# google-research/corenet

Hardware: AMD Instinct MI355X
Metric: voxels/sec fwd+bwd @128^3 (higher is better)
Workload: dtype bf16x3 (the convolutions of decoder stages 3-6 and the encoder's 3x3 convolutions -- forward of stages 4-5, data gradient of all -- multiply operands split into two bf16 terms: three bf16 MFMAs per product, fp32 accumulation, 16 mantissa bits, ~3e-6 relative per layer; tensors, everything else and t

## Files before the change

### corenet_amd/_lib.py

```python
from __future__ import annotations

import ctypes as C
import os
from typing import Optional

import torch as t

_HERE = os.path.dirname(os.path.abspath(__file__))
TOOLS_LIB_PATH = os.path.join(os.path.dirname(_HERE), "tools", "_build", "libcorenet_hip_tools.so")
PROBE_LIB_PATH = os.path.join(os.path.dirname(_HERE), "tools", "_build", "libcrn_probe.so")
LIB_PATH = os.environ.get("CORENET_HIP_LIB", TOOLS_LIB_PATH if os.environ.get("CRN_TOOLS_LIB") == "1" else
                          os.path.join(_HERE, "lib", "libcorenet_hip.so"))

c_i32p = C.POINTER(C.c_int32)
c_f32p = C.c_void_p
vp = C.c_void_p
i64 = C.c_int64
i32 = C.c_int
f32 = C.c_float
sz = C.c_size_t


class CrnTapBoxes(C.Structure):
  _fields_ = [("n_groups", C.c_int32), ("c_groups", C.c_int32), ("n_box", (C.c_int8 * 6) * 8),
# ... 32 lines not shown
  _fields_ = [("scale", vp), ("shift", vp), ("pre_relu", C.c_int32), ("post_relu", C.c_int32)]


class CrnBnBwdFuse(C.Structure):
  _fields_ = [("x", vp), ("sB_x", i64), ("saved", vp), ("pre_relu", C.c_int32), ("ws", vp), ("ws_bytes", sz),
              ("dsum", vp), ("ndsum", C.c_int32), ("nparts", C.c_int32)]


class HipError(RuntimeError):
  pass


_SIGS = {
    "crn_conv_fwd": [C.POINTER(CrnView), C.POINTER(CrnInTransform), vp, i32, vp, i32,
                     C.POINTER(CrnView), i32, i32, i32, i32, i32, i32, i32, i32, vp, vp],
    "crn_conv_fwd_plan": [C.POINTER(CrnView), C.POINTER(CrnInTransform), vp, i32, vp, i32,
                          C.POINTER(CrnView), i32, i32, i32, i32, i32, i32, i32, i32, vp, C.POINTER(CrnConvPlan)],
    "crn_conv_wgrad_plan": [C.POINTER(CrnView), C.POINTER(CrnInTransform), C.POINTER(CrnView), vp, i32,
                            i32, i32, i32, i32, i32, i32, i32, vp, C.POINTER(CrnConvPlan)],
    "crn_conv_fwd_bf3": [C.POINTER(CrnView), C.POINTER(CrnInTransform), vp, i32, vp, i32,
                         C.POINTER(CrnView), i32, i32, i32, i32, i32, i32, i32, vp, vp],
    "crn_conv_fwd_bf3_slabs": [C.POINTER(CrnView), C.POINTER(CrnInTransform), vp, i32, vp, i32,
                               C.POINTER(CrnView), i32, i32, i32, i32, i32, i32, i32, vp, vp],
    "crn_conv_fwd_bf3_slabs_bnbwd": [C.POINTER(CrnView), C.POINTER(CrnInTransform), vp, i32, vp, i32,
                                     C.POINTER(CrnView), i32, i32, i32, i32, i32, i32, i32, vp, C.POINTER(CrnBnBwdFuse), vp],
    "crn_conv_fwd_bf3_slabs_stats": [C.POINTER(CrnView), C.POINTER(CrnInTransform), vp, i32, vp, i32,
                                     C.POINTER(CrnView), i32, i32, i32, i32, i32, i32, i32, vp, i32, vp, sz, C.POINTER(C.c_int), vp],
    "crn_batch_renorm_bwd_apply": [vp, i64, vp, i64, i32, i32, i64, i32, vp, vp, vp, vp, vp, i64, vp, vp, i32, vp, i32,
                                   vp, sz, i32, vp],
    "crn_conv_wgrad_bf3": [C.POINTER(CrnView), C.POINTER(CrnInTransform), C.POINTER(CrnView), vp, i32,
# ... 250 lines not shown
```

### corenet_amd/backend.py

```python
from __future__ import annotations

import ctypes as C
from typing import Optional

import torch as t

from corenet_amd import _lib
from corenet_amd._lib import CrnInTransform, CrnView, ptr
from corenet_amd.views import View, space_to_depth_view, view_of

_DTYPE_CODE = {t.float32: 0, t.uint8: 1, t.int32: 2, t.float64: 3, t.int64: 4, t.int16: 5, t.int8: 6}


def _cview(v: View) -> CrnView:
  base = v.storage.data_ptr() + 4 * (v.offset - v.storage.storage_offset())
  c = v.__dict__.get("_crn")
  if c is None or c[0] != base:
    c = (base, CrnView(base, v.B, v.C, v.D, v.H, v.W, v.sB, v.sC, ptr(v.chan_off), v.sD, v.sH, v.sW))
    object.__setattr__(v, "_crn", c)
  return c[1]


class Transform:
  __slots__ = ("scale", "shift", "pre_relu", "post_relu")
# ... 52 lines not shown
               splits: int = 1, accumulate: bool = False, boxes=None, math: str = "fp32", wslab=None):
    if math == "bf16x3" and wslab is not None:
      self.lib.crn_conv_fwd_bf3_slabs(C.byref(_cview(x)), _ctr(tr), ptr(wslab), npad, ptr(bias), bias_sB,
                                      C.byref(_cview(y)), window[0], window[1], window[2],
                                      pad_lo[0], pad_lo[1], pad_lo[2], int(accumulate), _ctapboxes(boxes), _lib.stream())
      return
    if math == "bf16x3":
      self.lib.crn_conv_fwd_bf3(C.byref(_cview(x)), _ctr(tr), ptr(w), npad, ptr(bias), bias_sB,
                                C.byref(_cview(y)), window[0], window[1], window[2],
                                pad_lo[0], pad_lo[1], pad_lo[2], int(accumulate), _ctapboxes(boxes), _lib.stream())
      return
    self.lib.crn_conv_fwd(C.byref(_cview(x)), _ctr(tr), ptr(w), npad, ptr(bias), bias_sB,
                          C.byref(_cview(y)), window[0], window[1], window[2],
                          pad_lo[0], pad_lo[1], pad_lo[2], splits, int(accumulate), _ctapboxes(boxes),
                          _lib.stream())

  @staticmethod
  def _plan_dict(p) -> dict:
    d = {n: int(getattr(p, n)) for n, _ in p._fields_}
    d["path"] = _lib.PLAN_PATHS[d["path"]]
    return d

  def conv_fwd_plan(self, x: View, tr: Optional[Transform], w: t.Tensor, npad: int, bias: Optional[t.Tensor], bias_sB: int,
                    y: View, window, pad_lo, splits: int = 1, accumulate: bool = False, boxes=None) -> dict:
    p = _lib.CrnConvPlan()
    self.lib.crn_conv_fwd_plan(C.byref(_cview(x)), _ctr(tr), ptr(w), npad, ptr(bias), bias_sB, C.byref(_cview(y)),
                               window[0], window[1], window[2], pad_lo[0], pad_lo[1], pad_lo[2], splits, int(accumulate),
                               _ctapboxes(boxes), C.byref(p))
    return self._plan_dict(p)

# ... 452 lines not shown
```

### corenet_amd/csrc/batch_renorm.hip

```cpp
#include "crn_common.h"
#include <cstdlib>
#include <algorithm>
#include <type_traits>

namespace {

constexpr int kThreads = 256;

struct Slice { int64_t s0, s1; };
__device__ __forceinline__ Slice block_slice(int64_t S) {
  int64_t chunk = (S + gridDim.x - 1) / gridDim.x;
  chunk = (chunk + 3) & ~(int64_t)3;
  Slice r;
  r.s0 = (int64_t)blockIdx.x * chunk;
  r.s1 = min(S, r.s0 + chunk);
  return r;
}

template <bool VEC, typename F4, typename F1>
__device__ __forceinline__ void for_slice(Slice sl, F4 f4, F1 f1) {
  if (VEC) {
#pragma unroll 4
    for (int64_t s = sl.s0 + (int64_t)threadIdx.x * 4; s + 3 < sl.s1; s += (int64_t)kThreads * 4) f4(s);
    const int64_t nfull = (sl.s1 > sl.s0) ? ((sl.s1 - sl.s0) & ~(int64_t)3) : 0;
    for (int64_t s = sl.s0 + nfull + threadIdx.x; s < sl.s1; s += kThreads) f1(s);
  } else {
    for (int64_t s = sl.s0 + threadIdx.x; s < sl.s1; s += kThreads) f1(s);
  }
}

__device__ __forceinline__ void bn_acc(float v, int pre_relu, double& s1, double& s2) {
  if (pre_relu) v = fmaxf(v, 0.f);
  s1 += (double)v;
  s2 += (double)v * (double)v;
}

template <bool VEC>
__global__ __launch_bounds__(kThreads) void bn_partial_kernel(const float* x, int64_t S, int64_t sB,
                                                               int pre_relu, double* ws) {
  __shared__ double red[kThreads / 64];
  const int c = blockIdx.y, b = blockIdx.z;
  const float* p = x + (int64_t)b * sB + (int64_t)c * S;
  double s1 = 0.0, s2 = 0.0;
  auto one = [&](float v) { bn_acc(v, pre_relu, s1, s2); };
  for_slice<VEC>(block_slice(S),
                 [&](int64_t s) { const f32x4 v = *reinterpret_cast<const f32x4*>(p + s);
                                  one(v.x); one(v.y); one(v.z); one(v.w); },
                 [&](int64_t s) { one(p[s]); });
  const double t1 = crn_block_sum(s1, red);
  const double t2 = crn_block_sum(s2, red);
  if (threadIdx.x == 0) {
    const int nparts = gridDim.x * gridDim.z;
    double* o = ws + ((int64_t)c * nparts + (int64_t)b * gridDim.x + blockIdx.x) * 2;
    o[0] = t1; o[1] = t2;
  }
}

struct BnChannelIn { float g, bt, rmean, rvar, nt; };
__device__ __forceinline__ BnChannelIn bn_channel_in(int c, const float* gamma, const float* beta,
                                                     const float* running_mean, const float* running_var,
                                                     const int64_t* nbt) {
  return BnChannelIn{gamma[c], beta[c], running_mean[c], running_var[c], (float)nbt[0]};
}
// ... 90 lines not shown
    for_slice<VEC>(all,
                   [&](int64_t s) { const f32x4 v = *reinterpret_cast<const f32x4*>(p + s);
                                    one(v.x); one(v.y); one(v.z); one(v.w); },
                   [&](int64_t s) { one(p[s]); });
  }
  const double t1 = crn_block_sum(s1, red);
  const double t2 = crn_block_sum(s2, red);
  if (threadIdx.x == 0)
    bn_finalize_channel(c, C, t1, t2, (double)B * (double)S, cin, running_mean, running_var, eps, momentum, scale, shift,
                        saved);
}

typedef float f32x2 __attribute__((ext_vector_type(2)));

__device__ __forceinline__ f32x4 bn_splitk_sum(const float* part, int splits, int B, int C, int S4, int b, int c, int s4) {
  const f32x4* pp = reinterpret_cast<const f32x4*>(part) + ((int64_t)b * C + c) * S4 + s4;
  const int64_t slab4 = (int64_t)B * C * S4;
  f32x4 sum = (f32x4){0.f, 0.f, 0.f, 0.f};
  for (int sp = 0; sp < splits; ++sp) sum += pp[sp * slab4];
  return sum;
}

__device__ __forceinline__ bool bn_stride2_offset(int c, int s4, int W, int W2, int H2, int64_t& off) {
  const int s = s4 * 4, row = s / W, col = s - row * W;
  off = ((int64_t)c * H2 + (row >> 1)) * W2 + (col >> 1);
  return !(row & 1);
}

struct BnTail {
  const float* r; const float* rscale; const float* rshift; int64_t sBr;
  float* y_pre; int64_t sBpre; float* y; int64_t sBy; int relu;
  float* y2; int64_t sBy2; int W, W2, H2;
};
template <int NV, bool TAIL = false>
__global__ __launch_bounds__(kThreads) void bn_owner_stats_reg_kernel(
// ... 181 lines not shown
      f32x4 o;
#pragma unroll
      for (int i = 0; i < 4; ++i) {
        o[i] = bn_bwd_dx(xv[k][i], gv[k][i], pre_relu, post_relu, ch, kf, mg, mgx);
        lsum += o[i];
      }
      *reinterpret_cast<f32x4*>(dx + (int64_t)b * sBdx + ((int64_t)c * S4 + s4) * 4) = o;
    }
  }
  if (dsum && c < ndsum) {
    const float tsum = bn_block_sum_f32(lsum, redf);
    if (threadIdx.x == 0) dsum[c] = tsum;
  }
}

template <bool VEC>
__global__ __launch_bounds__(kThreads) void bn_bwd_partial_kernel(
    const float* x, int64_t sBx, const float* dy, int64_t sBdy, int64_t S, int C, int pre_relu,
    int post_relu, const float* scale, const float* shift, const float* saved, double* ws, float* dsum,
    int ndsum) {
  __shared__ double red[kThreads / 64];
  const int c = blockIdx.y, b = blockIdx.z;
  if (dsum && c < ndsum && blockIdx.x == 0 && b == 0 && threadIdx.x == 0) dsum[c] = 0.f;
  const float* px = x + (int64_t)b * sBx + (int64_t)c * S;
  const float* pg = dy + (int64_t)b * sBdy + (int64_t)c * S;
  const BnBwdChannel ch = bn_bwd_channel(c, C, scale, shift, saved);
  double s1 = 0.0, s2 = 0.0;
  auto one = [&](float xv, float gv) { bn_bwd_acc(xv, gv, pre_relu, post_relu, ch, s1, s2); };
  for_slice<VEC>(block_slice(S),
                 [&](int64_t s) { const f32x4 a = *reinterpret_cast<const f32x4*>(px + s);
                                  const f32x4 g = *reinterpret_cast<const f32x4*>(pg + s);
                                  one(a.x, g.x); one(a.y, g.y); one(a.z, g.z); one(a.w, g.w); },
                 [&](int64_t s) { one(px[s], pg[s]); });
  const double t1 = crn_block_sum(s1, red);
  const double t2 = crn_block_sum(s2, red);
  if (threadIdx.x == 0) {
    const int nparts = gridDim.x * gridDim.z;
    double* o = ws + ((int64_t)c * nparts + (int64_t)b * gridDim.x + blockIdx.x) * 2;
    o[0] = t1; o[1] = t2;
  }
}

template <bool VEC>
__global__ __launch_bounds__(kThreads) void bn_bwd_apply_kernel(
    const float* x, int64_t sBx, const float* dy, int64_t sBdy, int64_t S, int C, int pre_relu,
    int post_relu, const float* gamma, const float* scale, const float* shift, const float* saved,
    const double* ws, int nparts, double count, float* dx, int64_t sBdx, float* dgamma,
    float* dbeta, int accumulate, float* dsum, int ndsum) {
// ... 208 lines not shown

constexpr int kMaxParts = 64 * 64;

template <typename F>
inline void with_nv(int64_t BS, F f) {
  const int per = (int)crn_cdiv(BS / 4, kThreads);
  if (per <= 1) f(std::integral_constant<int, 1>{}); else if (per <= 2) f(std::integral_constant<int, 2>{});
  else if (per <= 4) f(std::integral_constant<int, 4>{}); else if (per <= 8) f(std::integral_constant<int, 8>{});
  else f(std::integral_constant<int, 16>{});
}
template <typename F>
inline void with_bool(bool on, F f) {
  if (on) f(std::true_type{}); else f(std::false_type{});
}

int take_or_flush_pending(const float* base, int64_t sB, int B, int C, int64_t S, hipStream_t st, bool reg_form,
                          const float** part, int* splits) {
  *part = nullptr; *splits = 0;
  CrnSplitPending& pend = crn_splitk_pending();
  if (!pend.active) return CRN_OK;
  const crnView& py = pend.y;
  if (reg_form && pend.stream == st && py.base == base && py.B == B && py.C == C && (int64_t)py.D * py.H * py.W == S && sB == (int64_t)C * S) {
    *part = pend.scratch; *splits = pend.splits; pend.active = false;
    return CRN_OK;
  }
  return crn_splitk_flush(st);
}

int bias_grad_ordered(const float* src, int B, int n, int64_t S, int64_t sB, int ns, float* out, int accumulate, double* ws,
                      size_t ws_bytes, hipStream_t st) {
  const int nparts = ns * B;
  if (ws_bytes < (size_t)n * nparts * sizeof(double)) return CRN_ENOMEM;
  with_bool(vec_ok(S, {sB}, {src}), [&](auto vec) {
    hipLaunchKernelGGL(bias_grad_partial_kernel<decltype(vec)::value>, dim3(ns, n, B), dim3(kThreads), 0, st, src, S, sB, ws);
  });
  CRN_CHECK_LAUNCH();
  hipLaunchKernelGGL(bias_grad_final_kernel, dim3(crn_cdiv(n, 4)), dim3(256), 0, st, ws, nparts, n, out, accumulate);
// ... 6 lines not shown
extern "C" size_t crn_batch_renorm_workspace_bytes(int C) {
  return (size_t)C * kMaxParts * 2 * sizeof(double);
}

static int bn_stats_impl(const float* x, int B, int C, int64_t S, int64_t sB, int pre_relu,
                         const float* gamma, const float* beta, float* running_mean,
                         float* running_var, const int64_t* nbt, float eps, float momentum,
                         int training, float* scale, float* shift, float* saved,
                         double* ws, size_t ws_bytes, crnStream stream, const BnTail* tail, bool* tail_done) {
  hipStream_t st = (hipStream_t)stream;
  if (B < 1 || C < 1 || S < 1 || B > 64) return CRN_EINVAL;
  if (!x || !gamma || !beta || !running_mean || !running_var || !scale || !shift) return CRN_EINVAL;
  if (training && (!nbt || !saved)) return CRN_EINVAL;
  int nparts = 1;
  const bool reg_form = training && owner_form(S, C, B) && vec_ok(S, {sB}, {x}) && (int64_t)B * S <= 16384;
  const float* part;
  int psplits;
  const int rcp = take_or_flush_pending(x, sB, B, C, S, st, reg_form, &part, &psplits);
  if (rcp != CRN_OK) return rcp;
  if (reg_form) {
    const bool with_tail = tail && vec_ok(S, {tail->r ? tail->sBr : 0, tail->y_pre ? tail->sBpre : 0, tail->y ? tail->sBy : 0},
                                          {tail->r, tail->y_pre, tail->y});
    with_nv((int64_t)B * S, [&](auto nv) {
      with_bool(with_tail, [&](auto fused) {
        hipLaunchKernelGGL((bn_owner_stats_reg_kernel<decltype(nv)::value, decltype(fused)::value>), dim3(C), dim3(kThreads), 0, st,
                           const_cast<float*>(x), B, C, (int)(S / 4), sB, pre_relu, gamma, beta, running_mean, running_var, nbt,
                           eps, momentum, scale, shift, saved, part, psplits, with_tail ? *tail : BnTail{});
      });
    });
    if (with_tail) *tail_done = true;
    CRN_CHECK_LAUNCH();
    return CRN_OK;
  }
  if (training && owner_form(S, C, B)) {
    with_bool(vec_ok(S, {sB}, {x}), [&](auto vec) {
      hipLaunchKernelGGL(bn_owner_stats_kernel<decltype(vec)::value>, dim3(C), dim3(kThreads), 0, st, x, B, C, S, sB, pre_relu,
                         gamma, beta, running_mean, running_var, nbt, eps, momentum, scale, shift, saved);
    });
    CRN_CHECK_LAUNCH();
    return CRN_OK;
  }
  if (training) {
    const int ns = nsplit_for(S, C, B);
    nparts = ns * B;
    if (ws_bytes < (size_t)C * nparts * 2 * sizeof(double)) return CRN_ENOMEM;
    dim3 grid(ns, C, B);
    with_bool(vec_ok(S, {sB}, {x}), [&](auto vec) {
      hipLaunchKernelGGL(bn_partial_kernel<decltype(vec)::value>, grid, dim3(kThreads), 0, st, x, S, sB, pre_relu, ws);
    });
    CRN_CHECK_LAUNCH();
  }
  hipLaunchKernelGGL(bn_finalize_kernel, dim3(crn_cdiv(C, 4)), dim3(256), 0, st, ws, nparts, C,
                     (double)B * (double)S, gamma, beta, running_mean, running_var, nbt, eps, momentum,
                     training, scale, shift, saved);
  CRN_CHECK_LAUNCH();
  return CRN_OK;
}

extern "C" int crn_batch_renorm_stats(const float* x, int B, int C, int64_t S, int64_t sB, int pre_relu,
                                      const float* gamma, const float* beta, float* running_mean,
                                      float* running_var, const int64_t* nbt, float eps, float momentum,
                                      int training, float* scale, float* shift, float* saved,
                                      double* ws, size_t ws_bytes, crnStream stream) {
// ... 89 lines not shown
    if (reg_form && hv) {
      with_nv((int64_t)B * S, [&](auto nv) {
        hipLaunchKernelGGL((bn_owner_bwd_reg_kernel<decltype(nv)::value, true>), dim3(C), dim3(kThreads), 0, st, x, sB_x, dy, sB_dy,
                           B, (int)(S / 4), C, pre_relu, post_relu, gamma, scale, shift, saved, dx, sB_dx, dgamma, dbeta,
                           accumulate, dsum, ndsum, (const float*)nullptr, 0, *head);
      });
      CRN_CHECK_LAUNCH();
      return CRN_OK;
    }
    const int rch = crn_relu_bwd_add_impl(head->g, head->act, head->g2, B, C, S, head->sBg, head->sBact, head->sBg2,
                                          const_cast<float*>(dy), sB_dy, stream);
    if (rch != CRN_OK) return rch;
  }
  const float* part;
  int psplits;
  const int rcp = take_or_flush_pending(dy, sB_dy, B, C, S, st, reg_form, &part, &psplits);
  if (rcp != CRN_OK) return rcp;
  if (reg_form) {
    with_nv((int64_t)B * S, [&](auto nv) {
      hipLaunchKernelGGL(bn_owner_bwd_reg_kernel<decltype(nv)::value>, dim3(C), dim3(kThreads), 0, st, x, sB_x, dy, sB_dy, B,
                         (int)(S / 4), C, pre_relu, post_relu, gamma, scale, shift, saved, dx, sB_dx, dgamma, dbeta, accumulate,
                         dsum, ndsum, part, psplits);
    });
    CRN_CHECK_LAUNCH();
    return CRN_OK;
  }
  if (owner_ok) {
    with_bool(v, [&](auto vec) {
      hipLaunchKernelGGL(bn_owner_bwd_kernel<decltype(vec)::value>, dim3(C), dim3(kThreads), 0, st, x, sB_x, dy, sB_dy, B, S, C,
                         pre_relu, post_relu, gamma, scale, shift, saved, dx, sB_dx, dgamma, dbeta, accumulate, dsum, ndsum);
    });
    CRN_CHECK_LAUNCH();
    return CRN_OK;
  }
  const int ns = nsplit_for(S, C, B);
  const int nparts = ns * B;
  if (ws_bytes < (size_t)C * nparts * 2 * sizeof(double)) return CRN_ENOMEM;
  dim3 grid(ns, C, B);
  float* const dsum_det = (dsum && ndsum > 0 && crn_deterministic()) ? dsum : nullptr;
  if (dsum_det) dsum = nullptr;
  with_bool(v, [&](auto vec) {
    hipLaunchKernelGGL(bn_bwd_partial_kernel<decltype(vec)::value>, grid, dim3(kThreads), 0, st, x, sB_x, dy, sB_dy, S, C,
                       pre_relu, post_relu, scale, shift, saved, ws, dsum, ndsum);
  });
  CRN_CHECK_LAUNCH();
  with_bool(v, [&](auto vec) {
    hipLaunchKernelGGL(bn_bwd_apply_kernel<decltype(vec)::value>, grid, dim3(kThreads), 0, st, x, sB_x, dy, sB_dy, S, C,
                       pre_relu, post_relu, gamma, scale, shift, saved, ws, nparts,
                       (double)B * (double)S, dx, sB_dx, dgamma, dbeta, accumulate, dsum, ndsum);
  });
  CRN_CHECK_LAUNCH();
  if (dsum_det) return bias_grad_ordered(dx, B, ndsum, S, sB_dx, ns, dsum_det, 0, ws, ws_bytes, st);
  return CRN_OK;
}

extern "C" int crn_batch_renorm_bwd(const float* x, int64_t sB_x, const float* dy, int64_t sB_dy,
                                    int B, int C, int64_t S, int pre_relu, int post_relu,
                                    const float* gamma, const float* scale, const float* shift,
// ... 103 lines not shown
```

### corenet_amd/csrc/conv_igemm.hip

```cpp
#include "conv_kernels.h"
#include <algorithm>
#include <cstring>
#include <cstdio>
#include <cstdlib>

namespace {
using namespace crnk;

struct PwGeom {
  const float* x; float* y; const float* w; const float* bias;
  crnInTransform tr;
  int B, C, N, Npad, S;
  int64_t xsB, ysB;
  int64_t ysC, ysP;
  int bias_sB, mode;
  int splits, cps;
  long long* stamps;
};

constexpr int kPwBN = 32;
constexpr int kPwTab = 2048;
template <int NS>
__global__ __launch_bounds__(256) void pointwise_fwd_kernel(PwGeom g) {
  constexpr int BM = 64, BN = NS * 16, KC = 64, SA = BM + 16, SB = BN + 16;
  constexpr int NRA = KC / 16;
  __shared__ __attribute__((aligned(16))) float ldsA[KC * SA];
  __shared__ __attribute__((aligned(16))) float ldsB[KC * SB];
  crn_kernargs_now(g.x, g.y, g.w, g.bias, g.tr.scale, g.tr.shift, g.tr.pre_relu, g.tr.post_relu, g.B, g.C, g.N, g.Npad,
                   g.S, g.xsB, g.ysB, g.ysC, g.ysP, g.bias_sB, g.mode, g.splits, g.cps);
  const long long t_entry = (long long)__builtin_amdgcn_s_memtime();
  const long long r_entry = (long long)__builtin_amdgcn_s_memrealtime();
  const int tid = threadIdx.x, lane = tid & 63, wave = tid >> 6;
  const int i16 = lane & 15, kk = lane >> 4;
  const int m0 = blockIdx.x * BM, n0 = blockIdx.y * BN;
  const bool stamp = g.stamps && blockIdx.x == 0 && blockIdx.y == 0 && blockIdx.z == 0 && tid == 0;
  int nmark = 0;
  auto mark = [&]() { if (stamp && nmark < 30) g.stamps[nmark] = (long long)__builtin_amdgcn_s_memtime() - t_entry; ++nmark; };
  mark();
  const int split = blockIdx.z / g.B, b = blockIdx.z - split * g.B;
  const int cbeg = split * g.cps, cend = min(g.C, cbeg + g.cps);
  const float* xb = g.x + (int64_t)b * g.xsB;
  const int ka = tid >> 4, ca = (tid & 15) * 4;
  constexpr int BQ = BN / 4, BROWS = 256 / BQ, NRB = KC / BROWS;
  const int kb = tid / BQ, cb = (tid % BQ) * 4;
  const bool a_ok = (m0 + ca) < g.S;
  const bool b_ok = (n0 + cb) < g.Npad;
  extern __shared__ float pw_tables[];
  const bool has_tr = g.tr.scale != nullptr;
  float* tsc = pw_tables; float* tsh = pw_tables + g.cps;
  constexpr unsigned kOOBo = 0x80000000u;
  constexpr int NL = NRA + NRB;
  const crn_rsrc xrs = crnk::make_rsrc(xb);
  const crn_rsrc wrs = crnk::make_rsrc(g.w);
  f32x4 ra[2][NRA], rb[2][NRB];
  auto issue = [&](int c0, f32x4 (&pa_)[NRA], f32x4 (&pb_)[NRB]) {
#pragma unroll
    for (int q = 0; q < NRA; ++q) {
      const int c_a = c0 + ka + q * 16;
      const unsigned off = (a_ok && c_a < cend) ? (unsigned)(c_a * g.S + m0 + ca) * 4u : kOOBo;
      crnk::crn_bload4(pa_[q], xrs, off);
    }
#pragma unroll
    for (int q = 0; q < NRB; ++q) {
      const int c_b = c0 + kb + q * BROWS;
      const unsigned off = (b_ok && c_b < cend) ? (unsigned)(c_b * g.Npad + n0 + cb) * 4u : kOOBo;
      crnk::crn_bload4(pb_[q], wrs, off);
    }
  };
  auto wait_slot = [&](f32x4 (&pa_)[NRA], f32x4 (&pb_)[NRB]) {
#pragma unroll
    for (int q = 0; q < NRA; ++q) asm volatile("s_waitcnt vmcnt(%1)" : "+v"(pa_[q]) : "n"(NL));
#pragma unroll
    for (int q = 0; q < NRB; ++q) asm volatile("s_waitcnt vmcnt(%1)" : "+v"(pb_[q]) : "n"(NL));
  };
  auto xform = [&](f32x4 v, int c) -> f32x4 {
    if (has_tr && a_ok && c < cend) {
      const float sc = tsc[c - cbeg], sh = tsh[c - cbeg];
#pragma unroll
      for (int i = 0; i < 4; ++i) {
        float t = v[i];
        if (g.tr.pre_relu) t = fmaxf(t, 0.f);
// ... 286 lines not shown
  int path;
  int zs;
  int pw_splits, pw_cps;
  int pw_cps_whole;
  FwdCfg cfg;
  int xvec, lead;
  bool forced;
  int splits, nchunks;
};

bool fwd_vec_store(const crnView& y, int mw, int mode) {
  return y.sW == 1 && mw >= 4 && (y.W & 3) == 0 && (y.sH & 3) == 0 && (y.sD & 3) == 0 && (y.sB & 3) == 0 &&
         (y.sC & 3) == 0 && (((uintptr_t)y.base) & 15) == 0 && y.chan_off == nullptr && mode != 2;
}

int fwd_select(const crnView* x, const crnInTransform* tr, const float* w, int Npad, const crnView* y,
               int kd, int kh, int kw, int pd, int ph, int pw, int splits, FwdSel* s) {
  *s = FwdSel{};
  const int64_t Sx = (int64_t)x->D * x->H * x->W;
  const bool has_scale = tr && tr->scale;
  if (kd * kh * kw == 1 && pd == 0 && ph == 0 && pw == 0 && splits <= 1 && one_position(*x) && one_position(*y) &&
      x->B <= kDenseB) {
    if (y->C >= 1024 && x->C <= 2048) { s->path = CRN_PLAN_DENSE_COLS; return CRN_OK; }
    if (y->C <= 256 && !has_scale && x->C >= 1024) {
      s->path = CRN_PLAN_DENSE_ROWS;
      s->zs = (y->sC == 1 && y->sB >= y->C && !crn_deterministic()) ? std::max(1, std::min(16, x->C / 2048)) : 1;
      return CRN_OK;
    }
  }
  if (kd * kh * kw == 1 && pd == 0 && ph == 0 && pw == 0 && splits <= 1 && plain_view(*x) && flat_out_view(*y) &&
      Sx == (int64_t)y->D * y->H * y->W && (Sx & 3) == 0 && (((uintptr_t)w) & 15) == 0 &&
      (int64_t)x->C * Sx * 4 < ((int64_t)1 << 31) && (int64_t)x->C * Npad * 4 < ((int64_t)1 << 31) &&
      (!has_scale || x->C <= kPwTab)) {
    s->path = CRN_PLAN_POINTWISE;
    s->pw_splits = 1; s->pw_cps = s->pw_cps_whole = (x->C + 63) & ~63;
    constexpr int pw_blocks = 256, pw_fill = 512, pw_minc = 128;
    const int64_t blocks = crn_cdiv(Sx, 64) * crn_cdiv(y->C, kPwBN) * (int64_t)x->B;
    if (splits < 1 && blocks < pw_blocks && x->C >= 2 * pw_minc) {
      int sp = (int)std::min<int64_t>(std::min<int64_t>(x->C / pw_minc, 16), crn_cdiv(pw_fill, blocks));
      if (sp > 1) {
        const int cps = (crn_cdiv(x->C, sp) + 31) & ~31;
        sp = crn_cdiv(x->C, cps);
        if (sp > 1) { s->pw_splits = sp; s->pw_cps = cps; }
        s->pw_cps_whole = (x->C + 31) & ~31;
      }
    }
    return CRN_OK;
  }
  s->path = CRN_PLAN_GENERIC;
  static const int kM[4] = {8, 4, 2, 1};
  static const int kN[3] = {4, 2, 1};
  const int xmode = vec_view(*x) ? 1 : ((x->sW == 2 && (x->W & 1) == 0) ? 2 : 0);
  g_stage_unit = xmode == 2 ? 2 : 4;
  const int lead = xmode == 1 ? vec_lead(pw) : (xmode == 2 ? ((pw % 2) + 2) % 2 : -1);
// ... 156 lines not shown
  }
  dim3 grid((unsigned)(g.tilesD * g.tilesH * g.tilesW * y->B), (unsigned)crn_cdiv(Npad, NSUB * 16),
            (unsigned)splits);
  const size_t lds_bytes = best.lds;
  g.vec_store = fwd_vec_store(*y, g.mw, g.mode) ? 1 : 0;
  if (boxes) {
    if (boxes->n_groups > 0 && y->C % boxes->n_groups == 0) { g.n_groups = boxes->n_groups; memcpy(g.n_box, boxes->n_box, sizeof(g.n_box)); }
    if (boxes->c_groups > 0 && x->C % boxes->c_groups == 0) { g.c_groups = boxes->c_groups; memcpy(g.c_box, boxes->c_box, sizeof(g.c_box)); }
  }
  int rc = CRN_EINVAL;
#define CRN_FWD_CASE(M, N) if (best.MSUB == M && NSUB == N) rc = crn_launch_fwd_##M##_##N(g, xvec, grid, lds_bytes, st);
  CRN_FWD_CONFIGS(CRN_FWD_CASE)
#undef CRN_FWD_CASE
  if (rc == CRN_OK && g.mode == 3) rc = crn_splitk_finish(yreal, scratch, splits, accumulate, armed, st);
  return rc;
}

namespace {
struct WgCand { int TD, TH, TW, RSUB, NSUB, CC, PW, PSP, POSP; double cost; size_t lds; };

bool wg_cand(int TD, int TH, int TW, int RSUB, int NSUB, int Cin, int Npad, int kd, int kh, int kw, int xlead,
             int dvec, size_t lds_budget, WgCand* out) {
  const int T = kd * kh * kw, NB = NSUB * 16, npos = TD * TH * TW;
  if (npos > 512 || RSUB * NSUB > 8 || (NSUB > 1 && NB > Npad)) return false;
  if ((xlead >= 0 || dvec) && (TW & 3)) return false;
  if (dvec == 1 ? (int64_t)NB * npos / 4 > 256 * NV
                : dvec == 2 ? (int64_t)NB * npos / 2 > 256 * NVX : stage_passes(NB, npos) > DREG) return false;
  const int PDp = TD + kd - 1, PH = TH + kh - 1, PW = patch_width(TW, kw, xlead), plane = PH * PW;
  int CC = std::min(std::min(std::max(1, (64 * RSUB) / T), Cin), 64);
  auto staged = [&](int cc) {
// ... 229 lines not shown
```

### corenet_amd/model/engine.py

```python
from __future__ import annotations

import dataclasses
import os
from typing import Dict, List, Optional, Tuple

import numpy as np
import torch as t

from corenet_amd import _lib
from corenet_amd import views as V
from corenet_amd.backend import Transform
from corenet_amd.model import conv_geometry as G

IMAGE_HW = (256, 256)


def check_image_hw(hw):
  H, W = int(hw[0]), int(hw[1])
  if H < 32 or W < 32 or H % 4 or W % 4 or H * W > 4096 * 4096:
    raise ValueError(f"corenet_amd.CoreNet: image batch of {H}x{W} pixels; this engine takes H and W that are multiples of 4 and >= 32 "
                     f"(256x256 in every shipped config)")
  return H, W
BN_EPS = 1e-3
BN_MOMENTUM = 0.01
# ... 745 lines not shown
          x, tr, cv.wop_f, g.npad, cv.bias, 0, y, g.window, g.pad_lo, accumulate))
      return
    self._timed("fwd   " + cv.name, lambda: self.be.conv_fwd(
        x, tr, cv.wf, g.npad, cv.bias, 0, y, g.window, g.pad_lo, 0, accumulate, boxes=(g.n_boxes, g.c_boxes),
        math=self._math(cv, "fwd"), wslab=cv.wop_f if cv.wop_kind == "slab" else None))

  def _dgrad(self, cv: Conv, dy: V.View, dx: V.View, accumulate=False):
    g = cv.dgrad
    if cv.wop_d is not None and cv.wop_kind == "e2d" and self._e2d_shape_ok(dx, g.window):
      self._timed("dgrad " + cv.name, lambda: self.be.conv2d_bf3(
          dy, None, cv.wop_d, g.npad, None, 0, dx, g.window, g.pad_lo, accumulate))
      return
    self._timed("dgrad " + cv.name, lambda: self.be.conv_fwd(
        dy, None, cv.wd, g.npad, None, 0, dx, g.window, g.pad_lo, 0, accumulate, boxes=(g.n_boxes, g.c_boxes),
        math=self._math(cv, "dgrad"), wslab=cv.wop_d if cv.wop_kind == "slab" else None))

  def _dgrad_bn_bwd(self, cv: Conv, dy: V.View, g: t.Tensor, x: t.Tensor, Cn: int, S: int, b, dx: t.Tensor, cprev: Conv) -> bool:
    be = self.be
    gvw = self.vw(g)
    fusable = (hasattr(be, "conv_dgrad_bn_bwd") and cv.wop_kind == "slab" and cv.wop_d is not None
               and self._math(cv, "dgrad") == "bf16x3")
    if not fusable:
      be.splitk_defer()
      self._dgrad(cv, dy, gvw)
      return False
    gd = cv.dgrad
    be.splitk_defer()
    return self._timed("dgrad " + cv.name, lambda: be.conv_dgrad_bn_bwd(
        dy, cv.wop_d, gd.npad, gvw, g, gd.window, gd.pad_lo, (gd.n_boxes, gd.c_boxes), x, Cn * S, self.B, Cn, S, True, b.gamma,
        b.scale, b.shift, b.saved, dx, Cn * S, b.dgamma, b.dbeta, dsum=cprev.dbias, ndsum=cprev.n_ref))
# ... 449 lines not shown
    self._dgrad(cc, self.vw(blk.gyc), self.vw(blk.gab))
    self._bn_bwd(bb, blk.yb, blk.gab, blk.gyb, S, False, True, bias_of=cb)
    self._wgrad(cb, self.vw(blk.ya), tra, self.vw(blk.gyb))
    be.splitk_defer()
    self._dgrad(cb, self.vw(blk.gyb), self.vw(blk.gaa))
    self._bn_bwd(ba, blk.ya, blk.gaa, blk.gya, S, False, True, bias_of=ca)
    xin = self.vw(blk.xs) if blk.stride == 2 else self.vw(blk.inp)
    self._wgrad(ca, xin, None, self.vw(blk.gya))
    if blk.down:
      bs = bn[p + "shortcut.bn."]
      csn = cv[p + "shortcut.conv."]
      self._bn_bwd(bs, blk.ys, gpre, blk.gys, S, False, False, bias_of=csn)
      self._wgrad(csn, xin, None, self.vw(blk.gys))
      gin = blk.gin
      gv = self.vw(blk.gxs) if blk.stride == 2 else self.vw(gin)
      self._dgrad(ca, self.vw(blk.gya), gv)
      self._dgrad(csn, self.vw(blk.gys), gv, accumulate=True)
      if blk.stride == 2:
        if hasattr(be, "bn_bwd_head"):
          self._g_compact = blk.gxs
        else:
          be.stride2_scatter(blk.gxs, gin)
      return gin
    self._dgrad(ca, self.vw(blk.gya), self.vw(gpre), accumulate=True)
    return gpre
```

### include/corenet_hip.h

```cpp
#ifndef CORENET_HIP_H_
#define CORENET_HIP_H_

#include <stddef.h>
#include <stdint.h>

#ifdef __cplusplus
extern "C" {
#endif

#define CRN_OK 0
#define CRN_EINVAL (-1)
#define CRN_ENOMEM (-2)
#define CRN_ENOCONV (-3)

typedef void* crnStream;

typedef struct {
  float* base;
  int32_t B, C, D, H, W;
  int64_t sB, sC;
  const int32_t* chan_off;
  int32_t sD, sH, sW;
} crnView;

// ... 2 lines not shown
  const float* shift;
  int32_t pre_relu, post_relu;
} crnInTransform;

typedef struct {
  int32_t n_groups, c_groups;
  int8_t n_box[8][6];
  int8_t c_box[8][6];
} crnTapBoxes;

int crn_conv_fwd(const crnView* x, const crnInTransform* tr, const float* w, int Npad,
                 const float* bias, int bias_sB, const crnView* y,
                 int kd, int kh, int kw, int pd, int ph, int pw,
                 int splits, int accumulate ,
                 const crnTapBoxes* boxes , crnStream stream);

#define CRN_PLAN_DENSE_COLS 1
#define CRN_PLAN_DENSE_ROWS 2
#define CRN_PLAN_DENSE_WGRAD 3
#define CRN_PLAN_POINTWISE 4
#define CRN_PLAN_GENERIC 5
typedef struct {
  int32_t path;
  int32_t msub, nsub;
  int32_t xstage, dystage;
  int32_t forced;
  int32_t cc;
  int32_t td, th, tw;
  int32_t mw;
  int32_t splits;
// ... 414 lines not shown
```

Measured before the change: 1.196 billion.

## Fuse paired 1x1 dgrad convs into one kernel and fold pending split-K into BN partials

Adds a paired pointwise forward kernel that computes both the block conv and shortcut conv data gradients for downsampling blocks in one launch, concatenating along the reduction dimension so no separate accumulate pass is needed. It also lets the non-owner BN partial kernels (forward and backward) consume pending split-K partial buffers directly, summing them and writing back the result instead of flushing them in a separate kernel. This is meant to cut kernel launches and an extra read/write of the output tensor. The cost is more template variants and extra logic in the inner loads.

```diff
diff --git a/corenet_amd/_lib.py b/corenet_amd/_lib.py
--- a/corenet_amd/_lib.py
+++ b/corenet_amd/_lib.py
@@ -70,6 +70,7 @@
 _SIGS = {
     "crn_conv_fwd": [C.POINTER(CrnView), C.POINTER(CrnInTransform), vp, i32, vp, i32,
                      C.POINTER(CrnView), i32, i32, i32, i32, i32, i32, i32, i32, vp, vp],
+    "crn_conv1x1_fwd_pair": [C.POINTER(CrnView), vp, C.POINTER(CrnView), vp, i32, C.POINTER(CrnView), i32, i32, vp],
     "crn_conv_fwd_plan": [C.POINTER(CrnView), C.POINTER(CrnInTransform), vp, i32, vp, i32,
                           C.POINTER(CrnView), i32, i32, i32, i32, i32, i32, i32, i32, vp, C.POINTER(CrnConvPlan)],
     "crn_conv_wgrad_plan": [C.POINTER(CrnView), C.POINTER(CrnInTransform), C.POINTER(CrnView), vp, i32,
diff --git a/corenet_amd/backend.py b/corenet_amd/backend.py
--- a/corenet_amd/backend.py
+++ b/corenet_amd/backend.py
@@ -90,6 +90,14 @@
                           C.byref(_cview(y)), window[0], window[1], window[2],
                           pad_lo[0], pad_lo[1], pad_lo[2], splits, int(accumulate), _ctapboxes(boxes),
                           _lib.stream())
+
+  def conv1x1_pair(self, x1: View, w1: t.Tensor, x2: View, w2: t.Tensor, npad: int, y: View, splits: int = 0,
+                   accumulate: bool = False) -> bool:
+    rc = self.lib._crn_conv1x1_fwd_pair(C.byref(_cview(x1)), ptr(w1), C.byref(_cview(x2)), ptr(w2), npad, C.byref(_cview(y)),
+                                        splits, int(accumulate), _lib.stream())
+    if rc not in (0, -1):
+      raise _lib.HipError(f"crn_conv1x1_fwd_pair failed with status {rc}")
+    return rc == 0
 
   @staticmethod
   def _plan_dict(p) -> dict:
diff --git a/corenet_amd/csrc/batch_renorm.hip b/corenet_amd/csrc/batch_renorm.hip
--- a/corenet_amd/csrc/batch_renorm.hip
+++ b/corenet_amd/csrc/batch_renorm.hip
@@ -29,24 +29,68 @@
   }
 }
 
+template <typename T>
+__device__ __forceinline__ T bn_splitk_sum_at(const T* p, int splits, int64_t slab) {
+  T sum = T{};
+  int sp = 0;
+  for (; sp + 4 <= splits; sp += 4) {
+    const T a = p[sp * slab], b = p[(sp + 1) * slab], c = p[(sp + 2) * slab], d = p[(sp + 3) * slab];
+    sum += a; sum += b; sum += c; sum += d;
+  }
+  const int rest = splits - sp;
+  if (rest > 0) {
+    const T a = p[sp * slab], b = rest > 1 ? p[(sp + 1) * slab] : T{}, c = rest > 2 ? p[(sp + 2) * slab] : T{};
+    sum += a;
+    if (rest > 1) sum += b;
+    if (rest > 2) sum += c;
+  }
+  return sum;
+}
+
+template <bool PEND>
+struct BnPendingRow {
+  const float* part; float* t; int64_t slab; int splits;
+  __device__ __forceinline__ f32x4 at4(int64_t o) const {
+    if (!PEND) return *reinterpret_cast<const f32x4*>(t + o);
+    const f32x4 v = bn_splitk_sum_at(reinterpret_cast<const f32x4*>(part + o), splits, slab / 4);
+    *reinterpret_cast<f32x4*>(t + o) = v;
+    return v;
+  }
+  __device__ __forceinline__ float at1(int64_t o) const {
+    if (!PEND) return t[o];
+    const float v = bn_splitk_sum_at(part + o, splits, slab);
+    t[o] = v;
+    return v;
+  }
+};
+template <bool PEND>
+__device__ __forceinline__ BnPendingRow<PEND> bn_pending_row(const float* t, int64_t sB, const float* part, int splits, int B,
+                                                             int C, int64_t S, int b, int c) {
+  BnPendingRow<PEND> r;
+  r.t = const_cast<float*>(t) + (int64_t)b * sB + (int64_t)c * S;
+  r.part = PEND ? part + ((int64_t)b * C + c) * S : nullptr;
+  r.slab = (int64_t)B * C * S; r.splits = splits;
+  return r;
+}
+
 __device__ __forceinline__ void bn_acc(float v, int pre_relu, double& s1, double& s2) {
   if (pre_relu) v = fmaxf(v, 0.f);
   s1 += (double)v;
   s2 += (double)v * (double)v;
 }
 
-template <bool VEC>
+template <bool VEC, bool PEND>
 __global__ __launch_bounds__(kThreads) void bn_partial_kernel(const float* x, int64_t S, int64_t sB,
-                                                               int pre_relu, double* ws) {
+                                                               int pre_relu, double* ws, const float* part, int splits) {
   __shared__ double red[kThreads / 64];
   const int c = blockIdx.y, b = blockIdx.z;
-  const float* p = x + (int64_t)b * sB + (int64_t)c * S;
+  const BnPendingRow<PEND> p = bn_pending_row<PEND>(x, sB, part, splits, gridDim.z, gridDim.y, S, b, c);
   double s1 = 0.0, s2 = 0.0;
   auto one = [&](float v) { bn_acc(v, pre_relu, s1, s2); };
   for_slice<VEC>(block_slice(S),
-                 [&](int64_t s) { const f32x4 v = *reinterpret_cast<const f32x4*>(p + s);
+                 [&](int64_t s) { const f32x4 v = p.at4(s);
                                   one(v.x); one(v.y); one(v.z); one(v.w); },
-                 [&](int64_t s) { one(p[s]); });
+                 [&](int64_t s) { one(p.at1(s)); });
   const double t1 = crn_block_sum(s1, red);
   const double t2 = crn_block_sum(s2, red);
   if (threadIdx.x == 0) {
@@ -167,11 +211,7 @@
 typedef float f32x2 __attribute__((ext_vector_type(2)));
 
 __device__ __forceinline__ f32x4 bn_splitk_sum(const float* part, int splits, int B, int C, int S4, int b, int c, int s4) {
-  const f32x4* pp = reinterpret_cast<const f32x4*>(part) + ((int64_t)b * C + c) * S4 + s4;
-  const int64_t slab4 = (int64_t)B * C * S4;
-  f32x4 sum = (f32x4){0.f, 0.f, 0.f, 0.f};
-  for (int sp = 0; sp < splits; ++sp) sum += pp[sp * slab4];
-  return sum;
+  return bn_splitk_sum_at(reinterpret_cast<const f32x4*>(part) + ((int64_t)b * C + c) * S4 + s4, splits, (int64_t)B * C * S4);
 }
 
 __device__ __forceinline__ bool bn_stride2_offset(int c, int s4, int W, int W2, int H2, int64_t& off) {
@@ -383,24 +423,24 @@
   }
 }
 
-template <bool VEC>
+template <bool VEC, bool PEND>
 __global__ __launch_bounds__(kThreads) void bn_bwd_partial_kernel(
     const float* x, int64_t sBx, const float* dy, int64_t sBdy, int64_t S, int C, int pre_relu,
     int post_relu, const float* scale, const float* shift, const float* saved, double* ws, float* dsum,
-    int ndsum) {
+    int ndsum, const float* part, int splits) {
   __shared__ double red[kThreads / 64];
   const int c = blockIdx.y, b = blockIdx.z;
   if (dsum && c < ndsum && blockIdx.x == 0 && b == 0 && threadIdx.x == 0) dsum[c] = 0.f;
   const float* px = x + (int64_t)b * sBx + (int64_t)c * S;
-  const float* pg = dy + (int64_t)b * sBdy + (int64_t)c * S;
+  const BnPendingRow<PEND> pg = bn_pending_row<PEND>(dy, sBdy, part, splits, gridDim.z, C, S, b, c);
   const BnBwdChannel ch = bn_bwd_channel(c, C, scale, shift, saved);
   double s1 = 0.0, s2 = 0.0;
   auto one = [&](float xv, float gv) { bn_bwd_acc(xv, gv, pre_relu, post_relu, ch, s1, s2); };
   for_slice<VEC>(block_slice(S),
                  [&](int64_t s) { const f32x4 a = *reinterpret_cast<const f32x4*>(px + s);
-                                  const f32x4 g = *reinterpret_cast<const f32x4*>(pg + s);
+                                  const f32x4 g = pg.at4(s);
                                   one(a.x, g.x); one(a.y, g.y); one(a.z, g.z); one(a.w, g.w); },
-                 [&](int64_t s) { one(px[s], pg[s]); });
+                 [&](int64_t s) { one(px[s], pg.at1(s)); });
   const double t1 = crn_block_sum(s1, red);
   const double t2 = crn_block_sum(s2, red);
   if (threadIdx.x == 0) {
@@ -639,13 +679,13 @@
   if (on) f(std::true_type{}); else f(std::false_type{});
 }
 
-int take_or_flush_pending(const float* base, int64_t sB, int B, int C, int64_t S, hipStream_t st, bool reg_form,
+int take_or_flush_pending(const float* base, int64_t sB, int B, int C, int64_t S, hipStream_t st, bool can_take,
                           const float** part, int* splits) {
   *part = nullptr; *splits = 0;
   CrnSplitPending& pend = crn_splitk_pending();
   if (!pend.active) return CRN_OK;
   const crnView& py = pend.y;
-  if (reg_form && pend.stream == st && py.base == base && py.B == B && py.C == C && (int64_t)py.D * py.H * py.W == S && sB == (int64_t)C * S) {
+  if (can_take && pend.stream == st && py.base == base && py.B == B && py.C == C && (int64_t)py.D * py.H * py.W == S && sB == (int64_t)C * S) {
     *part = pend.scratch; *splits = pend.splits; pend.active = false;
     return CRN_OK;
   }
@@ -682,9 +722,10 @@
   if (training && (!nbt || !saved)) return CRN_EINVAL;
   int nparts = 1;
   const bool reg_form = training && owner_form(S, C, B) && vec_ok(S, {sB}, {x}) && (int64_t)B * S <= 16384;
+  const bool two_pass = training && !owner_form(S, C, B) && ws_bytes >= (size_t)C * nsplit_for(S, C, B) * B * 2 * sizeof(double);
   const float* part;
   int psplits;
-  const int rcp = take_or_flush_pending(x, sB, B, C, S, st, reg_form, &part, &psplits);
+  const int rcp = take_or_flush_pending(x, sB, B, C, S, st, reg_form || two_pass, &part, &psplits);
   if (rcp != CRN_OK) return rcp;
   if (reg_form) {
     const bool with_tail = tail && vec_ok(S, {tail->r ? tail->sBr : 0, tail->y_pre ? tail->sBpre : 0, tail->y ? tail->sBy : 0},
@@ -714,7 +755,10 @@
     if (ws_bytes < (size_t)C * nparts * 2 * sizeof(double)) return CRN_ENOMEM;
     dim3 grid(ns, C, B);
     with_bool(vec_ok(S, {sB}, {x}), [&](auto vec) {
-      hipLaunchKernelGGL(bn_partial_kernel<decltype(vec)::value>, grid, dim3(kThreads), 0, st, x, S, sB, pre_relu, ws);
+      with_bool(part != nullptr, [&](auto pend) {
+        hipLaunchKernelGGL((bn_partial_kernel<decltype(vec)::value, decltype(pend)::value>), grid, dim3(kThreads), 0, st, x, S, sB,
+                           pre_relu, ws, part, psplits);
+      });
     });
     CRN_CHECK_LAUNCH();
   }
@@ -834,7 +878,8 @@
   }
   const float* part;
   int psplits;
-  const int rcp = take_or_flush_pending(dy, sB_dy, B, C, S, st, reg_form, &part, &psplits);
+  const bool two_pass = !owner_ok && ws_bytes >= (size_t)C * nsplit_for(S, C, B) * B * 2 * sizeof(double);
+  const int rcp = take_or_flush_pending(dy, sB_dy, B, C, S, st, reg_form || two_pass, &part, &psplits);
   if (rcp != CRN_OK) return rcp;
   if (reg_form) {
     with_nv((int64_t)B * S, [&](auto nv) {
@@ -860,8 +905,10 @@
   float* const dsum_det = (dsum && ndsum > 0 && crn_deterministic()) ? dsum : nullptr;
   if (dsum_det) dsum = nullptr;
   with_bool(v, [&](auto vec) {
-    hipLaunchKernelGGL(bn_bwd_partial_kernel<decltype(vec)::value>, grid, dim3(kThreads), 0, st, x, sB_x, dy, sB_dy, S, C,
-                       pre_relu, post_relu, scale, shift, saved, ws, dsum, ndsum);
+    with_bool(part != nullptr, [&](auto pend) {
+      hipLaunchKernelGGL((bn_bwd_partial_kernel<decltype(vec)::value, decltype(pend)::value>), grid, dim3(kThreads), 0, st, x, sB_x,
+                         dy, sB_dy, S, C, pre_relu, post_relu, scale, shift, saved, ws, dsum, ndsum, part, psplits);
+    });
   });
   CRN_CHECK_LAUNCH();
   with_bool(v, [&](auto vec) {
diff --git a/corenet_amd/csrc/conv_igemm.hip b/corenet_amd/csrc/conv_igemm.hip
--- a/corenet_amd/csrc/conv_igemm.hip
+++ b/corenet_amd/csrc/conv_igemm.hip
@@ -16,11 +16,14 @@
   int bias_sB, mode;
   int splits, cps;
   long long* stamps;
+  const float* x2; const float* w2;
+  int64_t x2sB;
+  int C1;
 };
 
 constexpr int kPwBN = 32;
 constexpr int kPwTab = 2048;
-template <int NS>
+template <int NS, bool PAIR = false>
 __global__ __launch_bounds__(256) void pointwise_fwd_kernel(PwGeom g) {
   constexpr int BM = 64, BN = NS * 16, KC = 64, SA = BM + 16, SB = BN + 16;
   constexpr int NRA = KC / 16;
@@ -28,6 +31,7 @@
   __shared__ __attribute__((aligned(16))) float ldsB[KC * SB];
   crn_kernargs_now(g.x, g.y, g.w, g.bias, g.tr.scale, g.tr.shift, g.tr.pre_relu, g.tr.post_relu, g.B, g.C, g.N, g.Npad,
                    g.S, g.xsB, g.ysB, g.ysC, g.ysP, g.bias_sB, g.mode, g.splits, g.cps);
+  if (PAIR) crn_kernargs_now(g.x2, g.w2, g.x2sB, g.C1);
   const long long t_entry = (long long)__builtin_amdgcn_s_memtime();
   const long long r_entry = (long long)__builtin_amdgcn_s_memrealtime();
   const int tid = threadIdx.x, lane = tid & 63, wave = tid >> 6;
@@ -52,19 +56,25 @@
   constexpr int NL = NRA + NRB;
   const crn_rsrc xrs = crnk::make_rsrc(xb);
   const crn_rsrc wrs = crnk::make_rsrc(g.w);
+  const crn_rsrc x2rs = crnk::make_rsrc(PAIR ? g.x2 + (int64_t)b * g.x2sB : xb);
+  const crn_rsrc w2rs = crnk::make_rsrc(PAIR ? g.w2 : g.w);
   f32x4 ra[2][NRA], rb[2][NRB];
   auto issue = [&](int c0, f32x4 (&pa_)[NRA], f32x4 (&pb_)[NRB]) {
+    const bool second = PAIR && c0 >= g.C1;
+    const crn_rsrc ars = second ? x2rs : xrs;
+    const crn_rsrc brs = second ? w2rs : wrs;
+    const int cs = second ? g.C1 : 0;
 #pragma unroll
     for (int q = 0; q < NRA; ++q) {
       const int c_a = c0 + ka + q * 16;
-      const unsigned off = (a_ok && c_a < cend) ? (unsigned)(c_a * g.S + m0 + ca) * 4u : kOOBo;
-      crnk::crn_bload4(pa_[q], xrs, off);
+      const unsigned off = (a_ok && c_a < cend) ? (unsigned)((c_a - cs) * g.S + m0 + ca) * 4u : kOOBo;
+      crnk::crn_bload4(pa_[q], ars, off);
     }
 #pragma unroll
     for (int q = 0; q < NRB; ++q) {
       const int c_b = c0 + kb + q * BROWS;
-      const unsigned off = (b_ok && c_b < cend) ? (unsigned)(c_b * g.Npad + n0 + cb) * 4u : kOOBo;
-      crnk::crn_bload4(pb_[q], wrs, off);
+      const unsigned off = (b_ok && c_b < cend) ? (unsigned)((c_b - cs) * g.Npad + n0 + cb) * 4u : kOOBo;
+      crnk::crn_bload4(pb_[q], brs, off);
     }
   };
   auto wait_slot = [&](f32x4 (&pa_)[NRA], f32x4 (&pb_)[NRB]) {
@@ -381,6 +391,12 @@
          (y.sC & 3) == 0 && (((uintptr_t)y.base) & 15) == 0 && y.chan_off == nullptr && mode != 2;
 }
 
+int pw_auto_splits(int C, int64_t blocks) {
+  constexpr int pw_blocks = 256, pw_fill = 512, pw_minc = 128;
+  if (blocks >= pw_blocks || C < 2 * pw_minc) return 1;
+  return (int)std::max<int64_t>(1, std::min<int64_t>(std::min<int64_t>(C / pw_minc, 16), crn_cdiv(pw_fill, blocks)));
+}
+
 int fwd_select(const crnView* x, const crnInTransform* tr, const float* w, int Npad, const crnView* y,
                int kd, int kh, int kw, int pd, int ph, int pw, int splits, FwdSel* s) {
   *s = FwdSel{};
@@ -401,10 +417,9 @@
       (!has_scale || x->C <= kPwTab)) {
     s->path = CRN_PLAN_POINTWISE;
     s->pw_splits = 1; s->pw_cps = s->pw_cps_whole = (x->C + 63) & ~63;
-    constexpr int pw_blocks = 256, pw_fill = 512, pw_minc = 128;
     const int64_t blocks = crn_cdiv(Sx, 64) * crn_cdiv(y->C, kPwBN) * (int64_t)x->B;
-    if (splits < 1 && blocks < pw_blocks && x->C >= 2 * pw_minc) {
-      int sp = (int)std::min<int64_t>(std::min<int64_t>(x->C / pw_minc, 16), crn_cdiv(pw_fill, blocks));
+    if (splits < 1) {
+      int sp = pw_auto_splits(x->C, blocks);
       if (sp > 1) {
         const int cps = (crn_cdiv(x->C, sp) + 31) & ~31;
         sp = crn_cdiv(x->C, cps);
@@ -591,6 +606,44 @@
 #undef CRN_FWD_CASE
   if (rc == CRN_OK && g.mode == 3) rc = crn_splitk_finish(yreal, scratch, splits, accumulate, armed, st);
   return rc;
+}
+
+extern "C" int crn_conv1x1_fwd_pair(const crnView* x1, const float* w1, const crnView* x2, const float* w2, int Npad,
+                                    const crnView* y, int splits, int accumulate, crnStream stream) {
+  if (!x1 || !x2 || !w1 || !w2 || !y || Npad <= 0 || (Npad & 15) || y->C > Npad || y->C < 1) return CRN_EINVAL;
+  if (!plain_view(*x1) || !plain_view(*x2) || !plain_view(*y)) return CRN_EINVAL;
+  const int64_t S = (int64_t)x1->D * x1->H * x1->W;
+  if ((int64_t)x2->D * x2->H * x2->W != S || (int64_t)y->D * y->H * y->W != S || (S & 3)) return CRN_EINVAL;
+  if (x1->B < 1 || x2->B != x1->B || y->B != x1->B || x1->C < 1 || (x1->C & 63) || x2->C < 1) return CRN_EINVAL;
+  if ((((uintptr_t)w1) & 15) || (((uintptr_t)w2) & 15)) return CRN_EINVAL;
+  constexpr int64_t kRange = (int64_t)1 << 31;
+  const int C1 = x1->C, C = C1 + x2->C;
+  if ((int64_t)std::max(C1, x2->C) * std::max<int64_t>(S, Npad) * 4 >= kRange || splits < 0) return CRN_EINVAL;
+  hipStream_t st = (hipStream_t)stream;
+  int rcf;
+  const bool armed = crn_splitk_begin(st, &rcf);
+  if (rcf != CRN_OK) return rcf;
+  int sp = splits;
+  if (sp == 0) sp = pw_auto_splits(C, crn_cdiv(S, 64) * crn_cdiv(y->C, kPwBN) * (int64_t)y->B);
+  sp = std::max(1, std::min(sp, C / 64));
+  int cps = (crn_cdiv(C, sp) + 63) & ~63;
+  sp = crn_cdiv(C, cps);
+  PwGeom p{};
+  p.x = x1->base; p.w = w1; p.x2 = x2->base; p.w2 = w2; p.y = y->base;
+  p.tr = crnInTransform{nullptr, nullptr, 0, 0};
+  p.B = y->B; p.C = C; p.C1 = C1; p.N = y->C; p.Npad = Npad; p.S = (int)S;
+  p.xsB = x1->sB; p.x2sB = x2->sB; p.ysB = y->sB; p.ysC = y->sC; p.ysP = 1; p.mode = accumulate ? 1 : 0;
+  p.splits = 1; p.cps = (C + 63) & ~63;
+  const int64_t ytot = (int64_t)y->B * y->C * S;
+  float* scratch = nullptr;
+  if (sp > 1 && (scratch = crn_splitk_scratch((size_t)sp * ytot, st)) != nullptr) {
+    p.splits = sp; p.cps = cps;
+    p.y = scratch; p.ysB = (int64_t)y->C * S; p.ysC = S; p.mode = 0;
+  }
+  dim3 grid((unsigned)crn_cdiv(S, 64), (unsigned)crn_cdiv(y->C, kPwBN), (unsigned)(y->B * p.splits));
+  hipLaunchKernelGGL((pointwise_fwd_kernel<kPwBN / 16, true>), grid, dim3(256), 0, st, p);
+  CRN_CHECK_LAUNCH();
+  return p.splits > 1 ? crn_splitk_finish(*y, scratch, p.splits, accumulate, armed, st) : CRN_OK;
 }
 
 namespace {
diff --git a/corenet_amd/model/engine.py b/corenet_amd/model/engine.py
--- a/corenet_amd/model/engine.py
+++ b/corenet_amd/model/engine.py
@@ -783,6 +783,15 @@
     self._timed("dgrad " + cv.name, lambda: self.be.conv_fwd(
         dy, None, cv.wd, g.npad, None, 0, dx, g.window, g.pad_lo, 0, accumulate, boxes=(g.n_boxes, g.c_boxes),
         math=self._math(cv, "dgrad"), wslab=cv.wop_d if cv.wop_kind == "slab" else None))
+
+  def _dgrad_pair(self, c1: Conv, dy1: V.View, c2: Conv, dy2: V.View, dx: V.View) -> bool:
+    be = self.be
+    g1, g2 = c1.dgrad, c2.dgrad
+    if (getattr(be, "conv1x1_pair", None) is None or self._math(c1, "dgrad") != "fp32" or self._math(c2, "dgrad") != "fp32"
+        or any(tuple(g.window) != (1, 1, 1) or any(g.pad_lo) for g in (g1, g2)) or g1.npad != g2.npad):
+      return False
+    return self._timed("dgrad " + c1.name + " + " + c2.name,
+                       lambda: be.conv1x1_pair(dy1, c1.wd, dy2, c2.wd, g1.npad, dx))
 
   def _dgrad_bn_bwd(self, cv: Conv, dy: V.View, g: t.Tensor, x: t.Tensor, Cn: int, S: int, b, dx: t.Tensor, cprev: Conv) -> bool:
     be = self.be
@@ -1262,8 +1271,9 @@
       self._wgrad(csn, xin, None, self.vw(blk.gys))
       gin = blk.gin
       gv = self.vw(blk.gxs) if blk.stride == 2 else self.vw(gin)
-      self._dgrad(ca, self.vw(blk.gya), gv)
-      self._dgrad(csn, self.vw(blk.gys), gv, accumulate=True)
+      if not self._dgrad_pair(ca, self.vw(blk.gya), csn, self.vw(blk.gys), gv):
+        self._dgrad(ca, self.vw(blk.gya), gv)
+        self._dgrad(csn, self.vw(blk.gys), gv, accumulate=True)
       if blk.stride == 2:
         if hasattr(be, "bn_bwd_head"):
           self._g_compact = blk.gxs
diff --git a/include/corenet_hip.h b/include/corenet_hip.h
--- a/include/corenet_hip.h
+++ b/include/corenet_hip.h
@@ -40,6 +40,9 @@
                  int kd, int kh, int kw, int pd, int ph, int pw,
                  int splits, int accumulate ,
                  const crnTapBoxes* boxes , crnStream stream);
+
+int crn_conv1x1_fwd_pair(const crnView* x1, const float* w1, const crnView* x2, const float* w2, int Npad,
+                         const crnView* y, int splits, int accumulate , crnStream stream);
 
 #define CRN_PLAN_DENSE_COLS 1
 #define CRN_PLAN_DENSE_ROWS 2
```

Result: faster. 1.208 billion (median of 6 runs) (+1.0%).
